# mishapadidar/GP-Derivatives-Variational-Inference

Hardware: AMD Instinct MI355X
Metric: ELBO steps/sec, DSVGP d=20 N=1M M=500 p=5 (higher is better)
Workload: dtype f32 (f64 Cholesky/solves); 1 GPU; DSVGP d=20 N=1M M=500 p=5 B=4096; global_batch=4096, per_gpu_batch=4096, M_prime=3000, parallelism=dp1 rows, trsm_nb=4096, graph_replay=False, one_call_step=True, dense_product=hand-written (gemm32.hip, v_mfma_f32_32x32x2_f32)

## Files before the change

gp-derivatives-variational-inference_amd/csrc/gemm32.hip:

```cpp
#include <type_traits>

#include "common.h"

namespace {

using acc16 = float __attribute__((ext_vector_type(16)));
using acc4f = float __attribute__((ext_vector_type(4)));
constexpr int TM = 128, TN = 128;

#ifndef G32_BK
#define G32_BK 32
#endif
#ifndef G32_MINW
#define G32_MINW 3
#endif
#ifndef G32_BAND
#define G32_BAND 8
#endif
#ifndef G32_DMA_BK
#define G32_DMA_BK 32
#endif
#ifndef G32_MF
#define G32_MF 32
#endif
#ifndef G32_SK_BELOW
#define G32_SK_BELOW 4096
#endif
#ifndef G32_SK_MINK
#define G32_SK_MINK 512
#endif
#ifndef G32_SK_SLOTS
#define G32_SK_SLOTS 256
#endif

struct G32 {
    const float* A; const float* B; float* C;
    int64_t lda, ldb, ldc;
    int M, N, K, tiles_m, tiles_n, flags, splitk, kslice, ntiles;
    float alpha;
    float* slab;
};

template <int BK, bool KC>
struct Stage {
    static constexpr int NV = BK / 8;
    float4 v[NV];
};

template <int BK>
struct FetchKC {
    static constexpr int CPR = BK / 4, RPP = 256 / CPR, NV = BK / 8;
    const float* P;
    int rowoff[NV];
    int kc, klim;
    __device__ __forceinline__ void init(const float* P_, int64_t ld, int mn0, int MN, int K, int tid) {
        P = P_;
        kc = (tid % CPR) * 4;
        klim = ((K + 3) / 4) * 4 - 4;
#pragma unroll
        for (int i = 0; i < NV; ++i) rowoff[i] = (int)(min(mn0 + tid / CPR + i * RPP, MN - 1) * ld);
    }
    __device__ __forceinline__ void load(int k0, int kend, Stage<BK, true>& s) const {
        const int k = k0 + kc;
        const float* p = P + min(k, klim);
#pragma unroll
        for (int i = 0; i < NV; ++i) s.v[i] = *reinterpret_cast<const float4*>(p + rowoff[i]);
        if (k0 + BK > kend) {
#pragma unroll
            for (int i = 0; i < NV; ++i) {
                s.v[i].x = (k < kend) ? s.v[i].x : 0.f;
                s.v[i].y = (k + 1 < kend) ? s.v[i].y : 0.f;
                s.v[i].z = (k + 2 < kend) ? s.v[i].z : 0.f;
                s.v[i].w = (k + 3 < kend) ? s.v[i].w : 0.f;
            }
        }
    }
};
template <int BK>
struct FetchMC {
    static constexpr int NV = BK / 8;
    const float* P;
    int64_t ld;
    int kr, K;
    __device__ __forceinline__ void init(const float* P_, int64_t ld_, int mn0, int MN, int K_, int tid) {
        ld = ld_; K = K_;
        kr = tid >> 5;
        P = P_ + min(mn0 + (tid & 31) * 4, ((MN + 3) / 4) * 4 - 4);
    }
    __device__ __forceinline__ void load(int k0, int kend, Stage<BK, false>& s) const {
#pragma unroll
        for (int i = 0; i < NV; ++i) {
            const int k = k0 + kr + 8 * i;
            s.v[i] = *reinterpret_cast<const float4*>(P + (int64_t)min(k, K - 1) * ld);
            if (k0 + BK > kend && k >= kend) s.v[i] = float4{0.f, 0.f, 0.f, 0.f};
        }
    }
};

__device__ __forceinline__ bool pick_unit(const G32& g, int& m0, int& n0, int& kbeg, int& kend) {
    const int u = (blockIdx.x >> 3) + (blockIdx.x & 7) * ((gridDim.x + 7) >> 3);
    if (u >= g.ntiles * g.splitk) return false;
    const int slice = u / g.ntiles;
    const int t = u - slice * g.ntiles;
    int tm, tn;
    if (g.flags & DSVGP_GEMM_OUT_LOWER) {
        const int tri = min(g.tiles_m, g.tiles_n), t0 = tri * (tri + 1) / 2;
        if (t < t0) {
            tm = (int)((sqrtf(8.f * (float)t + 1.f) - 1.f) * 0.5f);
            while ((tm + 1) * (tm + 2) / 2 <= t) ++tm;
            while (tm * (tm + 1) / 2 > t) --tm;
            tn = t - tm * (tm + 1) / 2;
        } else {
            tm = tri + (t - t0) / g.tiles_n;
            tn = (t - t0) % g.tiles_n;
        }
    } else {
        const int band = t / (G32_BAND * g.tiles_m), q = t - band * G32_BAND * g.tiles_m;
        const int wcols = min(G32_BAND, g.tiles_n - band * G32_BAND);
        tm = q / wcols;
        tn = band * G32_BAND + q - tm * wcols;
    }
    m0 = tm * TM; n0 = tn * TN;
    kbeg = slice * g.kslice; kend = min(g.K, kbeg + g.kslice);
    return true;
}

__device__ __forceinline__ void store_tile(const G32& g, const acc16 (&acc)[2][2], int m0, int n0, int wr, int wc, int h, int r,
                                           float* Cb, int64_t ldcb, bool atomic_) {
    const bool atomic = atomic_, out_lower = g.flags & DSVGP_GEMM_OUT_LOWER;
#pragma unroll
    for (int i = 0; i < 2; ++i)
#pragma unroll
        for (int j = 0; j < 2; ++j)
#pragma unroll
            for (int c = 0; c < 16; ++c) {
                const int m = m0 + wr * 64 + i * 32 + (c & 3) + 8 * (c >> 2) + 4 * h;
                const int n = n0 + wc * 64 + j * 32 + r;
                if (m >= g.M || n >= g.N) continue;
                if (out_lower && n > m) continue;
                const float v = g.alpha * acc[i][j][c];
                float* dst = Cb + (int64_t)m * ldcb + n;
                if (atomic) atomicAdd(dst, v);
                else *dst = v;
            }
}
#define G32_DEST()                                                                                     \
    const int slice_ = g.kslice > 0 ? kbeg / g.kslice : 0;                                             \
    float* const Cb = g.slab ? g.slab + (int64_t)slice_ * g.M * g.N : g.C;                            \
    const int64_t ldcb = g.slab ? (int64_t)g.N : g.ldc;                                                \
    const bool atomic_ = g.splitk > 1 && !g.slab

template <int BK, bool A_KC, bool B_KC>
__global__ __launch_bounds__(256, G32_MINW) void gemm32_kernel(const G32 g) {
    constexpr int SKC = BK + 2, SMC = TM + 4;
    constexpr int A_WORDS = A_KC ? TM * SKC : BK * SMC, B_WORDS = B_KC ? TN * SKC : BK * SMC;
    __shared__ __attribute__((aligned(16))) float lds[A_WORDS + B_WORDS];
    float* As = lds;
    float* Bs = lds + A_WORDS;
    const int tid = threadIdx.x, lane = tid & 63, wave = tid >> 6, wr = wave >> 1, wc = wave & 1;
    const int h = lane >> 5, r = lane & 31;
    int m0, n0, kbeg, kend;
    if (!pick_unit(g, m0, n0, kbeg, kend)) return;

    Stage<BK, A_KC> ra;
    Stage<BK, B_KC> rb;
    typename std::conditional<A_KC, FetchKC<BK>, FetchMC<BK>>::type fa;
    typename std::conditional<B_KC, FetchKC<BK>, FetchMC<BK>>::type fb;
    fa.init(g.A, g.lda, m0, g.M, g.K, tid);
    fb.init(g.B, g.ldb, n0, g.N, g.K, tid);
    auto fetch = [&](int k0) {
        fa.load(k0, kend, ra);
        fb.load(k0, kend, rb);
    };
    auto commit = [&]() {
        if constexpr (A_KC) {
            constexpr int CPR = BK / 4, RPP = 256 / CPR;
            float* p = As + (tid / CPR) * SKC + (tid % CPR) * 4;
#pragma unroll
            for (int i = 0; i < BK / 8; ++i) {
                *reinterpret_cast<float2*>(p + i * RPP * SKC) = float2{ra.v[i].x, ra.v[i].y};
                *reinterpret_cast<float2*>(p + i * RPP * SKC + 2) = float2{ra.v[i].z, ra.v[i].w};
            }
        } else {
            float* p = As + (tid >> 5) * SMC + (tid & 31) * 4;
#pragma unroll
            for (int i = 0; i < BK / 8; ++i) *reinterpret_cast<float4*>(p + 8 * i * SMC) = ra.v[i];
        }
        if constexpr (B_KC) {
            constexpr int CPR = BK / 4, RPP = 256 / CPR;
            float* p = Bs + (tid / CPR) * SKC + (tid % CPR) * 4;
#pragma unroll
            for (int i = 0; i < BK / 8; ++i) {
                *reinterpret_cast<float2*>(p + i * RPP * SKC) = float2{rb.v[i].x, rb.v[i].y};
                *reinterpret_cast<float2*>(p + i * RPP * SKC + 2) = float2{rb.v[i].z, rb.v[i].w};
            }
        } else {
            float* p = Bs + (tid >> 5) * SMC + (tid & 31) * 4;
#pragma unroll
            for (int i = 0; i < BK / 8; ++i) *reinterpret_cast<float4*>(p + 8 * i * SMC) = rb.v[i];
        }
    };

    acc16 acc[2][2];
#pragma unroll
    for (int i = 0; i < 2; ++i)
#pragma unroll
        for (int j = 0; j < 2; ++j)
#pragma unroll
            for (int c = 0; c < 16; ++c) acc[i][j][c] = 0.f;

    const float* af = A_KC ? As + (wr * 64 + r) * SKC + 2 * h : As + (2 * h) * SMC + wr * 64 + r;
    const float* bf = B_KC ? Bs + (wc * 64 + r) * SKC + 2 * h : Bs + (2 * h) * SMC + wc * 64 + r;

    if (kbeg < kend) {
        fetch(kbeg);
        for (int k0 = kbeg; k0 < kend; k0 += BK) {
            commit();
            __syncthreads();
            if (k0 + BK < kend) fetch(k0 + BK);
#pragma unroll
            for (int kk = 0; kk < BK / 4; ++kk) {
                float2 a[2], b[2];
#pragma unroll
                for (int i = 0; i < 2; ++i) {
                    if constexpr (A_KC) a[i] = *reinterpret_cast<const float2*>(af + i * 32 * SKC + 4 * kk);
                    else a[i] = float2{af[(4 * kk) * SMC + i * 32], af[(4 * kk + 1) * SMC + i * 32]};
                }
#pragma unroll
                for (int j = 0; j < 2; ++j) {
                    if constexpr (B_KC) b[j] = *reinterpret_cast<const float2*>(bf + j * 32 * SKC + 4 * kk);
                    else b[j] = float2{bf[(4 * kk) * SMC + j * 32], bf[(4 * kk + 1) * SMC + j * 32]};
                }
#pragma unroll
                for (int i = 0; i < 2; ++i)
#pragma unroll
                    for (int j = 0; j < 2; ++j) {
                        acc[i][j] = __builtin_amdgcn_mfma_f32_32x32x2f32(a[i].x, b[j].x, acc[i][j], 0, 0, 0);
                        acc[i][j] = __builtin_amdgcn_mfma_f32_32x32x2f32(a[i].y, b[j].y, acc[i][j], 0, 0, 0);
                    }
            }
            __syncthreads();
        }
    }

    G32_DEST();
    store_tile(g, acc, m0, n0, wr, wc, h, r, Cb, ldcb, atomic_);
}

#ifdef G32_STAMP
__device__ unsigned long long g32_stamps[8];
#define G32_T(var) unsigned long long var; do { __builtin_amdgcn_sched_barrier(0); \
    asm volatile("s_memtime %0\n\ts_waitcnt lgkmcnt(0)" : "=s"(var) :: "memory"); __builtin_amdgcn_sched_barrier(0); } while (0)
#else
#define G32_T(var) do { } while (0)
#endif
typedef __attribute__((address_space(3))) void* lds_ptr_t;
typedef const __attribute__((address_space(1))) void* glb_ptr_t;
__device__ __attribute__((aligned(16))) float g32_zero_chunk[4] = {0.f, 0.f, 0.f, 0.f};

__device__ __forceinline__ void lds_dma16(const float* gsrc, unsigned lds_byte_addr) {
    unsigned keep;
    asm volatile("s_mov_b32 %0, m0\n\ts_mov_b32 m0, %2\n\ts_nop 0\n\tglobal_load_lds_dwordx4 %1, off\n\ts_mov_b32 m0, %0"
                 : "=&s"(keep) : "v"(gsrc), "s"(lds_byte_addr) : "memory");
}

template <int MF, bool A_KC, bool B_KC, int BK>
__global__ __launch_bounds__(256, BK == 16 ? 3 : 2) void gemm32_dma_kernel(const G32 g) {
    static_assert(BK == 32 || (BK == 16 && MF == 32), "the 64-byte-row swizzle is derived for the 32 x 32 x 2 shape");
    constexpr int OPW = 128 * BK;
    constexpr int NP = BK / 8;
    constexpr int CH = BK / 4, RPP = 256 / BK;
    constexpr int TS = MF, NT = 64 / TS, NH = 64 / TS, NJ = BK / (4 * NH);
    __shared__ __attribute__((aligned(16))) float lds[2][2 * OPW];
    const int tid = threadIdx.x, lane = tid & 63, wave = tid >> 6, wr = wave >> 1, wc = wave & 1;
    const int h = lane / TS, r = lane % TS;
    int m0, n0, kbeg, kend;
    if (!pick_unit(g, m0, n0, kbeg, kend)) return;

    const float* asrc[NP];
    const float* bsrc[NP];
    int akk[NP], bkk[NP];
    const int K4 = (g.K + 3) / 4 * 4;
    auto swz = [](int R) { return BK == 32 ? ((R >> 1) & 7) : ((R >> 2) & 3); };
#pragma unroll
    for (int i = 0; i < NP; ++i) {
        const int blk = wave * NP + i;
        if constexpr (A_KC) {
            const int R = blk * RPP + lane / CH, c = (lane % CH) ^ swz(R);
            asrc[i] = g.A + (int64_t)min(m0 + R, g.M - 1) * g.lda + kbeg + 4 * c;
            akk[i] = 4 * c;
        } else {
            const int k = blk * 2 + (lane >> 5);
            asrc[i] = g.A + (int64_t)(kbeg + k) * g.lda + min(m0 + 4 * (lane & 31), (g.M + 3) / 4 * 4 - 4);
            akk[i] = k;
        }
        if constexpr (B_KC) {
            const int R = blk * RPP + lane / CH, c = (lane % CH) ^ swz(R);
            bsrc[i] = g.B + (int64_t)min(n0 + R, g.N - 1) * g.ldb + kbeg + 4 * c;
            bkk[i] = 4 * c;
        } else {
            const int k = blk * 2 + (lane >> 5);
            bsrc[i] = g.B + (int64_t)(kbeg + k) * g.ldb + min(n0 + 4 * (lane & 31), (g.N + 3) / 4 * 4 - 4);
            bkk[i] = k;
        }
    }
    const int64_t astep = A_KC ? BK : (int64_t)BK * g.lda, bstep = B_KC ? BK : (int64_t)BK * g.ldb;
    const unsigned lds_base = (unsigned)(uintptr_t)(lds_ptr_t)&lds[0][0];
    const unsigned wave_u = __builtin_amdgcn_readfirstlane(wave);
    auto dma = [&](int buf, int k0) {
        const unsigned dst = lds_base + (unsigned)buf * (2 * OPW * 4) + wave_u * (NP * 1024);
        const bool tail = k0 + BK > kend;
#pragma unroll
        for (int i = 0; i < NP; ++i) {
            const float* sa = asrc[i];
            const float* sb = bsrc[i];
            if (tail) {
                if (k0 + akk[i] >= (A_KC ? K4 : g.K)) sa = g32_zero_chunk;
                if (k0 + bkk[i] >= (B_KC ? K4 : g.K)) sb = g32_zero_chunk;
            }
            lds_dma16(sa, dst + i * 1024);
            lds_dma16(sb, dst + OPW * 4 + i * 1024);
            asrc[i] += astep;
            bsrc[i] += bstep;
        }
    };

    using accT = typename std::conditional<MF == 32, acc16, acc4f>::type;
    accT acc[NT][NT];
#pragma unroll
    for (int i = 0; i < NT; ++i)
#pragma unroll
        for (int j = 0; j < NT; ++j)
#pragma unroll
            for (int c = 0; c < (MF == 32 ? 16 : 4); ++c) acc[i][j][c] = 0.f;

    const int q7 = h ^ swz(r);
    int aoff[NJ], boff[NJ];
#pragma unroll
    for (int j = 0; j < NJ; ++j) {
        aoff[j] = A_KC ? (wr * 64 + r) * BK + 4 * ((NH * j) ^ q7) : (4 * NH * j + 4 * h) * 128 + wr * 64 + r;
        boff[j] = B_KC ? (wc * 64 + r) * BK + 4 * ((NH * j) ^ q7) : (4 * NH * j + 4 * h) * 128 + wc * 64 + r;
    }

    struct Frag { float a[NT][4], b[NT][4]; };
    auto load_frag = [&](const float* As, const float* Bs, int j, Frag& f) {
#pragma unroll
        for (int i = 0; i < NT; ++i) {
            if constexpr (A_KC) {
                const float4 v = *reinterpret_cast<const float4*>(As + aoff[j] + i * TS * BK);
                f.a[i][0] = v.x; f.a[i][1] = v.y; f.a[i][2] = v.z; f.a[i][3] = v.w;
            } else {
#pragma unroll
                for (int e = 0; e < 4; ++e) f.a[i][e] = As[aoff[j] + e * 128 + i * TS];
            }
            if constexpr (B_KC) {
                const float4 v = *reinterpret_cast<const float4*>(Bs + boff[j] + i * TS * BK);
                f.b[i][0] = v.x; f.b[i][1] = v.y; f.b[i][2] = v.z; f.b[i][3] = v.w;
            } else {
#pragma unroll
                for (int e = 0; e < 4; ++e) f.b[i][e] = Bs[boff[j] + e * 128 + i * TS];
            }
        }
    };

    if (kbeg < kend) {
        dma(0, kbeg);
        asm volatile("s_waitcnt vmcnt(0)" ::: "memory");
        __syncthreads();
        int buf = 0;
#ifdef G32_STAMP
        unsigned long long d_dma = 0, d_mfma = 0, d_vm = 0, d_bar = 0, n_st = 0;
#endif
        for (int k0 = kbeg; k0 < kend; k0 += BK, buf ^= 1) {
            G32_T(t0);
            if (k0 + BK < kend) dma(buf ^ 1, k0 + BK);
            G32_T(t1);
            const float* As = &lds[buf][0];
            const float* Bs = As + OPW;
            Frag f[2];
            load_frag(As, Bs, 0, f[0]);
#pragma unroll
            for (int j = 0; j < NJ; ++j) {
                if (j + 1 < NJ) load_frag(As, Bs, j + 1, f[(j + 1) & 1]);
                __builtin_amdgcn_sched_barrier(0);
                const Frag& c = f[j & 1];
#pragma unroll
                for (int e = 0; e < 4; ++e)
#pragma unroll
                    for (int i = 0; i < NT; ++i)
#pragma unroll
                        for (int jn = 0; jn < NT; ++jn) {
                            if constexpr (MF == 32)
                                acc[i][jn] = __builtin_amdgcn_mfma_f32_32x32x2f32(c.a[i][e], c.b[jn][e], acc[i][jn], 0, 0, 0);
                            else
                                acc[i][jn] = __builtin_amdgcn_mfma_f32_16x16x4f32(c.a[i][e], c.b[jn][e], acc[i][jn], 0, 0, 0);
                        }
                __builtin_amdgcn_sched_barrier(0);
            }
            G32_T(t2);
            asm volatile("s_waitcnt vmcnt(0)" ::: "memory");
            G32_T(t3);
            __syncthreads();
#ifdef G32_STAMP
            G32_T(t4);
            d_dma += t1 - t0; d_mfma += t2 - t1; d_vm += t3 - t2; d_bar += t4 - t3; ++n_st;
#endif
        }
#ifdef G32_STAMP
        if (tid == 0 && blockIdx.x == gridDim.x / 2 + 8) {
            g32_stamps[0] = d_dma; g32_stamps[1] = d_mfma; g32_stamps[2] = d_vm; g32_stamps[3] = d_bar; g32_stamps[4] = n_st;
        }
#endif
    }
    G32_DEST();
    if constexpr (MF == 32) {
        store_tile(g, acc, m0, n0, wr, wc, h, r, Cb, ldcb, atomic_);
    } else {
        const bool atomic = atomic_, out_lower = g.flags & DSVGP_GEMM_OUT_LOWER;
#pragma unroll
        for (int i = 0; i < NT; ++i)
#pragma unroll
            for (int j = 0; j < NT; ++j)
#pragma unroll
                for (int c = 0; c < 4; ++c) {
                    const int m = m0 + wr * 64 + i * 16 + 4 * h + c;
                    const int n = n0 + wc * 64 + j * 16 + r;
                    if (m >= g.M || n >= g.N) continue;
                    if (out_lower && n > m) continue;
                    const float v = g.alpha * acc[i][j][c];
                    float* dst = Cb + (int64_t)m * ldcb + n;
                    if (atomic) atomicAdd(dst, v);
                    else *dst = v;
                }
    }
}

template <int BK>
int dispatch32(hipStream_t st, const G32& a, dim3 grid, bool akc, bool bkc) {
    if (akc && bkc) hipLaunchKernelGGL((gemm32_kernel<BK, true, true>), grid, dim3(256), 0, st, a);
    else if (akc) hipLaunchKernelGGL((gemm32_kernel<BK, true, false>), grid, dim3(256), 0, st, a);
    else if (bkc) hipLaunchKernelGGL((gemm32_kernel<BK, false, true>), grid, dim3(256), 0, st, a);
    else hipLaunchKernelGGL((gemm32_kernel<BK, false, false>), grid, dim3(256), 0, st, a);
    hipError_t e = hipGetLastError();
    return e == hipSuccess ? 1 : 1000 + (int)e;
}

}

#ifdef G32_STAMP
int g32_read_stamps(unsigned long long* out) { return (int)hipMemcpyFromSymbol(out, HIP_SYMBOL(g32_stamps), sizeof(unsigned long long) * 8); }
#endif

int launch_gemm32(hipStream_t st, const GemmArgs& g) {
    const int fl = g.flags;
    if (fl & ~(DSVGP_GEMM_TRANS_A | DSVGP_GEMM_TRANS_B | DSVGP_GEMM_OUT_LOWER | DSVGP_GEMM_K_PADDED | DSVGP_GEMM_C_ZEROED | DSVGP_GEMM_UPPER_UNDEF)) return 0;
    if (g.batch != 1 || g.splitk != 1 || g.Cin || g.kscale || g.C32 || !g.C || g.beta != 0.0) return 0;
    if (g.M < 512 || g.N < 512 || g.K < 512) return 0;
    if (g.lda % 4 || g.ldb % 4 || ((uintptr_t)g.A % 16) || ((uintptr_t)g.B % 16)) return 0;
    {
        const int64_t a_minor = (fl & DSVGP_GEMM_TRANS_A) ? g.M : g.K, b_minor = (fl & DSVGP_GEMM_TRANS_B) ? g.K : g.N;
        if (g.lda < (a_minor + 3) / 4 * 4 || g.ldb < (b_minor + 3) / 4 * 4) return 0;
        const int64_t a_rows = (fl & DSVGP_GEMM_TRANS_A) ? g.K : g.M, b_rows = (fl & DSVGP_GEMM_TRANS_B) ? g.N : g.K;
        if (a_rows * g.lda >= (int64_t)1 << 31 || b_rows * g.ldb >= (int64_t)1 << 31) return 0;
    }
    const bool out_lower = fl & DSVGP_GEMM_OUT_LOWER;
    G32 a{};
    a.A = (const float*)g.A; a.B = (const float*)g.B; a.C = (float*)g.C;
    a.lda = g.lda; a.ldb = g.ldb; a.ldc = g.ldc;
    a.M = g.M; a.N = g.N; a.K = g.K; a.flags = fl; a.alpha = (float)g.alpha;
    a.tiles_m = cdiv(g.M, TM); a.tiles_n = cdiv(g.N, TN);
    if (out_lower) {
        const int tri = a.tiles_m < a.tiles_n ? a.tiles_m : a.tiles_n;
        a.ntiles = tri * (tri + 1) / 2 + (a.tiles_m > tri ? (a.tiles_m - tri) * a.tiles_n : 0);
    } else {
        a.ntiles = a.tiles_m * a.tiles_n;
    }
    int sk = 1;
    if (a.ntiles < G32_SK_BELOW && g.K >= G32_SK_MINK) {
        double best = 1e300;
        const int maxsk = g.K / 256 < 64 ? g.K / 256 : 64;
        for (int c = 1; c <= maxsk; ++c) {
            const double tcost = (double)cdiv((int64_t)a.ntiles * c, G32_SK_SLOTS) * ((double)g.K / c + 384.0);
            if (tcost < best * 0.999) { best = tcost; sk = c; }
        }
    }
    sk = slab_slices(g, sk, sizeof(float));
    a.splitk = sk;
    a.kslice = cdiv(cdiv(g.K, sk), 32) * 32;
    a.splitk = cdiv(g.K, a.kslice);
    a.slab = (g.slab && a.splitk > 1) ? (float*)g.slab : nullptr;
    if (!a.slab && (a.splitk > 1 || (out_lower && !(fl & DSVGP_GEMM_UPPER_UNDEF))) && !(fl & DSVGP_GEMM_C_ZEROED)) {
        hipError_t e = zero_block(a.C, sizeof(float), a.ldc, a.M, a.N, st);
        if (e != hipSuccess) return 1000 + (int)e;
    }
    const dim3 grid(cdiv((int64_t)a.ntiles * a.splitk, 8) * 8);
    const bool akc = !(fl & DSVGP_GEMM_TRANS_A), bkc = (fl & DSVGP_GEMM_TRANS_B) != 0;
    if (!((akc || bkc) && g.K % 4 != 0 && !(g.flags & DSVGP_GEMM_K_PADDED))) {
        if (akc && bkc) hipLaunchKernelGGL((gemm32_dma_kernel<G32_MF, true, true, G32_DMA_BK>), grid, dim3(256), 0, st, a);
        else if (akc) hipLaunchKernelGGL((gemm32_dma_kernel<G32_MF, true, false, G32_DMA_BK>), grid, dim3(256), 0, st, a);
        else if (bkc) hipLaunchKernelGGL((gemm32_dma_kernel<G32_MF, false, true, G32_DMA_BK>), grid, dim3(256), 0, st, a);
        else hipLaunchKernelGGL((gemm32_dma_kernel<G32_MF, false, false, G32_DMA_BK>), grid, dim3(256), 0, st, a);
        hipError_t e = hipGetLastError();
        if (e != hipSuccess) return 1000 + (int)e;
    } else
    {
        const int rc = dispatch32<G32_BK>(st, a, grid, akc, bkc);
        if (rc != 1) return rc;
    }
    if (a.slab) {
        const int rc = launch_splitk_reduce(st, 0, a.slab, a.splitk, a.M, a.N, a.C, a.ldc, nullptr, 0, out_lower ? 1 : 0, 0);
        if (rc) return rc;
    }
    return 1;
}
```

Before: 83.69 steps/s.

## Add wide 256x192-tile fp32 MFMA GEMM kernel for large non-split GEMMs

Adds a new GEMM kernel with a 256x192 output tile per block, one block per CU, double-buffered LDS DMA loads and MFMA issue interleaved with LDS reads and DMA via sched barriers. A heuristic selects it for non-transposed-A, transposed-B-free, non-lower, non-slab GEMMs with enough tiles to fill several rounds at high occupancy fill. The larger tile raises arithmetic intensity and cuts global/LDS traffic per flop, at the cost of lower occupancy and possible tail imbalance. An environment variable can force or disable it.

```diff
diff --git a/gp-derivatives-variational-inference_amd/csrc/gemm32.hip b/gp-derivatives-variational-inference_amd/csrc/gemm32.hip
--- a/gp-derivatives-variational-inference_amd/csrc/gemm32.hip
+++ b/gp-derivatives-variational-inference_amd/csrc/gemm32.hip
@@ -1,3 +1,4 @@
+#include <cstdlib>
 #include <type_traits>
 
 #include "common.h"
@@ -28,6 +29,12 @@
 #endif
 #ifndef G32_SK_MINK
 #define G32_SK_MINK 512
+#endif
+#ifndef G32_WIDE_ROUNDS
+#define G32_WIDE_ROUNDS 3
+#endif
+#ifndef G32_WIDE_FILL
+#define G32_WIDE_FILL 90
 #endif
 #ifndef G32_SK_SLOTS
 #define G32_SK_SLOTS 256
@@ -97,6 +104,7 @@
     }
 };
 
+template <int TM_ = TM, int TN_ = TN>
 __device__ __forceinline__ bool pick_unit(const G32& g, int& m0, int& n0, int& kbeg, int& kend) {
     const int u = (blockIdx.x >> 3) + (blockIdx.x & 7) * ((gridDim.x + 7) >> 3);
     if (u >= g.ntiles * g.splitk) return false;
@@ -120,22 +128,23 @@
         tm = q / wcols;
         tn = band * G32_BAND + q - tm * wcols;
     }
-    m0 = tm * TM; n0 = tn * TN;
+    m0 = tm * TM_; n0 = tn * TN_;
     kbeg = slice * g.kslice; kend = min(g.K, kbeg + g.kslice);
     return true;
 }
 
-__device__ __forceinline__ void store_tile(const G32& g, const acc16 (&acc)[2][2], int m0, int n0, int wr, int wc, int h, int r,
+template <int NI, int NJ>
+__device__ __forceinline__ void store_tile(const G32& g, const acc16 (&acc)[NI][NJ], int m0, int n0, int wr, int wc, int h, int r,
                                            float* Cb, int64_t ldcb, bool atomic_) {
     const bool atomic = atomic_, out_lower = g.flags & DSVGP_GEMM_OUT_LOWER;
 #pragma unroll
-    for (int i = 0; i < 2; ++i)
-#pragma unroll
-        for (int j = 0; j < 2; ++j)
+    for (int i = 0; i < NI; ++i)
+#pragma unroll
+        for (int j = 0; j < NJ; ++j)
 #pragma unroll
             for (int c = 0; c < 16; ++c) {
-                const int m = m0 + wr * 64 + i * 32 + (c & 3) + 8 * (c >> 2) + 4 * h;
-                const int n = n0 + wc * 64 + j * 32 + r;
+                const int m = m0 + wr * (32 * NI) + i * 32 + (c & 3) + 8 * (c >> 2) + 4 * h;
+                const int n = n0 + wc * (32 * NJ) + j * 32 + r;
                 if (m >= g.M || n >= g.N) continue;
                 if (out_lower && n > m) continue;
                 const float v = g.alpha * acc[i][j][c];
@@ -435,6 +444,136 @@
     }
 }
 
+constexpr int WTM = 256, WTN = 192, WBK = 32;
+constexpr int W_AWORDS = WTM * WBK, W_BWORDS = WBK * WTN, W_STAGE = W_AWORDS + W_BWORDS;
+constexpr int W_NA = W_AWORDS / 1024, W_NB = W_BWORDS / 1024;
+constexpr int W_LDS_BYTES = 2 * W_STAGE * 4;
+
+__global__ __launch_bounds__(256, 1) void gemm32_wide_kernel(const G32 g) {
+    extern __shared__ __attribute__((aligned(16))) float wlds[];
+    const int tid = threadIdx.x, lane = tid & 63, wave = tid >> 6, wr = wave >> 1, wc = wave & 1;
+    const int h = lane >> 5, r = lane & 31;
+    int m0, n0, kbeg, kend;
+    if (!pick_unit<WTM, WTN>(g, m0, n0, kbeg, kend)) return;
+
+    const float* asrc[W_NA];
+    const float* bsrc[W_NB];
+    int akk[W_NA], bkk[W_NB];
+    const int K4 = (g.K + 3) / 4 * 4;
+#pragma unroll
+    for (int i = 0; i < W_NA; ++i) {
+        const int R = (wave * W_NA + i) * 8 + (lane >> 3), c = (lane & 7) ^ ((R >> 1) & 7);
+        asrc[i] = g.A + (int64_t)min(m0 + R, g.M - 1) * g.lda + kbeg + 4 * c;
+        akk[i] = 4 * c;
+    }
+#pragma unroll
+    for (int i = 0; i < W_NB; ++i) {
+        const int ch = (wave * W_NB + i) * 64 + lane, k = ch / (WTN / 4), n4 = ch % (WTN / 4);
+        bsrc[i] = g.B + (int64_t)(kbeg + k) * g.ldb + min(n0 + 4 * n4, (g.N + 3) / 4 * 4 - 4);
+        bkk[i] = k;
+    }
+    const int64_t bstep = (int64_t)WBK * g.ldb;
+    const unsigned lds_base = (unsigned)(uintptr_t)(lds_ptr_t)&wlds[0];
+    const unsigned wave_u = __builtin_amdgcn_readfirstlane(wave);
+
+    acc16 acc[4][3];
+#pragma unroll
+    for (int i = 0; i < 4; ++i)
+#pragma unroll
+        for (int j = 0; j < 3; ++j)
+#pragma unroll
+            for (int c = 0; c < 16; ++c) acc[i][j][c] = 0.f;
+
+    const int q7 = h ^ ((r >> 1) & 7);
+    int aoff[4];
+#pragma unroll
+    for (int j = 0; j < 4; ++j) aoff[j] = (wr * 128 + r) * WBK + 4 * ((2 * j) ^ q7);
+    const int boff = (4 * h) * WTN + wc * 96 + r;
+
+    auto stage = [&](auto mode_, int buf, int knext) {
+        constexpr int MODE = decltype(mode_)::value;
+        const float* As = wlds + buf * W_STAGE;
+        const float* Bs = As + W_AWORDS;
+        const unsigned dst = lds_base + (unsigned)(buf ^ 1) * (W_STAGE * 4);
+        float fa[2][4][4], fb[2][3][4];
+        auto rd_a = [&](int j, int i) {
+            const float4 v = *reinterpret_cast<const float4*>(As + aoff[j] + i * 32 * WBK);
+            fa[j & 1][i][0] = v.x; fa[j & 1][i][1] = v.y; fa[j & 1][i][2] = v.z; fa[j & 1][i][3] = v.w;
+        };
+        auto rd_b = [&](int j, int jn, int ep) {
+#pragma unroll
+            for (int e = 2 * ep; e < 2 * ep + 2; ++e) fb[j & 1][jn][e] = Bs[boff + (8 * j + e) * WTN + jn * 32];
+        };
+        auto dma1 = [&](int d) {
+            if (d < W_NA) {
+                const float* s = asrc[d];
+                if (MODE == 2) s = (knext + akk[d] >= K4) ? g32_zero_chunk : s;
+                lds_dma16(s, dst + (wave_u * W_NA + d) * 1024);
+                asrc[d] += WBK;
+            } else {
+                const int i = d - W_NA;
+                const float* s = bsrc[i];
+                if (MODE == 2) s = (knext + bkk[i] >= g.K) ? g32_zero_chunk : s;
+                lds_dma16(s, dst + W_AWORDS * 4 + (wave_u * W_NB + i) * 1024);
+                bsrc[i] += bstep;
+            }
+        };
+#pragma unroll
+        for (int i = 0; i < 4; ++i) rd_a(0, i);
+#pragma unroll
+        for (int q = 0; q < 6; ++q) rd_b(0, q >> 1, q & 1);
+#pragma unroll
+        for (int j = 0; j < 4; ++j) {
+            const int nd = MODE == 0 ? 0 : (j < 2 ? 5 : (j == 2 ? 4 : 0)), d0 = j < 2 ? 5 * j : 10;
+#pragma unroll
+            for (int n = 0; n < 48; ++n) {
+                const int e = n / 12, i = (n / 3) % 4, jn = n % 3;
+                acc[i][jn] = __builtin_amdgcn_mfma_f32_32x32x2f32(fa[j & 1][i][e], fb[j & 1][jn][e], acc[i][jn], 0, 0, 0);
+                if (n & 1) {
+                    const int t = n >> 1;
+                    __builtin_amdgcn_sched_barrier(0);
+                    if (t < nd) {
+                        dma1(d0 + t);
+                    } else if (j < 3) {
+                        const int q = t - nd;
+                        if (q < 4) rd_a(j + 1, q);
+                        else if (q < 10) rd_b(j + 1, (q - 4) >> 1, (q - 4) & 1);
+                    }
+                    __builtin_amdgcn_sched_barrier(0);
+                }
+            }
+        }
+        if (MODE != 0) {
+            asm volatile("s_waitcnt vmcnt(0)" ::: "memory");
+            __syncthreads();
+        }
+    };
+
+    if (kbeg < kend) {
+        const int nst = (kend - kbeg + WBK - 1) / WBK;
+        {
+            const unsigned dst = lds_base;
+#pragma unroll
+            for (int i = 0; i < W_NA; ++i) {
+                lds_dma16((kbeg + akk[i] >= K4) ? g32_zero_chunk : asrc[i], dst + (wave_u * W_NA + i) * 1024);
+                asrc[i] += WBK;
+            }
+#pragma unroll
+            for (int i = 0; i < W_NB; ++i) {
+                lds_dma16((kbeg + bkk[i] >= g.K) ? g32_zero_chunk : bsrc[i], dst + W_AWORDS * 4 + (wave_u * W_NB + i) * 1024);
+                bsrc[i] += bstep;
+            }
+        }
+        asm volatile("s_waitcnt vmcnt(0)" ::: "memory");
+        __syncthreads();
+        int buf = 0, k0 = kbeg + WBK;
+        for (int s = 0; s + 2 < nst; ++s, buf ^= 1, k0 += WBK) stage(std::integral_constant<int, 1>{}, buf, k0);
+        if (nst >= 2) { stage(std::integral_constant<int, 2>{}, buf, k0); buf ^= 1; }
+        stage(std::integral_constant<int, 0>{}, buf, 0);
+    }
+    store_tile(g, acc, m0, n0, wr, wc, h, r, g.C, g.ldc, false);
+}
+
 template <int BK>
 int dispatch32(hipStream_t st, const G32& a, dim3 grid, bool akc, bool bkc) {
     if (akc && bkc) hipLaunchKernelGGL((gemm32_kernel<BK, true, true>), grid, dim3(256), 0, st, a);
@@ -484,6 +623,31 @@
             if (tcost < best * 0.999) { best = tcost; sk = c; }
         }
     }
+    const bool akc = !(fl & DSVGP_GEMM_TRANS_A), bkc = (fl & DSVGP_GEMM_TRANS_B) != 0;
+    const bool dma_ok = !((akc || bkc) && g.K % 4 != 0 && !(g.flags & DSVGP_GEMM_K_PADDED));
+    const char* wenv = getenv("DSVGP_G32_WIDE");
+    const int wmode = wenv ? atoi(wenv) : 3;
+    const bool wide_can = !out_lower && akc && !bkc && dma_ok && !g.slab;
+    bool wide = false;
+    if (wmode == 3) {
+        const int64_t wt = (int64_t)cdiv(g.M, WTM) * cdiv(g.N, WTN), rounds = (wt + G32_SK_SLOTS - 1) / G32_SK_SLOTS;
+        wide = wide_can && sk == 1 && wt >= (int64_t)G32_WIDE_ROUNDS * G32_SK_SLOTS && wt * 100 >= rounds * G32_SK_SLOTS * G32_WIDE_FILL;
+    } else if (wmode != 0) {
+        if (wmode == 2 && !wide_can) return 1000 + (int)hipErrorInvalidValue;
+        if (wide_can) sk = 1;
+        wide = wide_can && wmode > 0;
+    }
+    if (wide) {
+        a.tiles_m = cdiv(g.M, WTM); a.tiles_n = cdiv(g.N, WTN);
+        a.ntiles = a.tiles_m * a.tiles_n;
+        a.splitk = 1;
+        a.kslice = cdiv(g.K, 32) * 32;
+        hipError_t e = hipFuncSetAttribute((const void*)gemm32_wide_kernel, hipFuncAttributeMaxDynamicSharedMemorySize, W_LDS_BYTES);
+        if (e != hipSuccess) return 1000 + (int)e;
+        hipLaunchKernelGGL(gemm32_wide_kernel, dim3(cdiv(a.ntiles, 8) * 8), dim3(256), W_LDS_BYTES, st, a);
+        e = hipGetLastError();
+        return e == hipSuccess ? 1 : 1000 + (int)e;
+    }
     sk = slab_slices(g, sk, sizeof(float));
     a.splitk = sk;
     a.kslice = cdiv(cdiv(g.K, sk), 32) * 32;
@@ -494,8 +658,7 @@
         if (e != hipSuccess) return 1000 + (int)e;
     }
     const dim3 grid(cdiv((int64_t)a.ntiles * a.splitk, 8) * 8);
-    const bool akc = !(fl & DSVGP_GEMM_TRANS_A), bkc = (fl & DSVGP_GEMM_TRANS_B) != 0;
-    if (!((akc || bkc) && g.K % 4 != 0 && !(g.flags & DSVGP_GEMM_K_PADDED))) {
+    if (dma_ok) {
         if (akc && bkc) hipLaunchKernelGGL((gemm32_dma_kernel<G32_MF, true, true, G32_DMA_BK>), grid, dim3(256), 0, st, a);
         else if (akc) hipLaunchKernelGGL((gemm32_dma_kernel<G32_MF, true, false, G32_DMA_BK>), grid, dim3(256), 0, st, a);
         else if (bkc) hipLaunchKernelGGL((gemm32_dma_kernel<G32_MF, false, true, G32_DMA_BK>), grid, dim3(256), 0, st, a);
```

After: 85.76 steps/s, median of 6. 1.02x the previous value.
